# MaurizioFD/RecSys2019_DeepLearning_Evaluation

Hardware: NVIDIA H100
Metric: ItemKNN cosine top-K rows/sec (higher is better)
Workload: dtype i32 counts + f32

## Files before the change

recsys2019_deeplearning_evaluation_b200/csrc/sim_k1d.cuh:

```cuda

constexpr int D_THREADS = 512;
constexpr int D_WARPS = D_THREADS / 32;
constexpr int D_ROWS = 4;
constexpr int D_TILE_LOG2 = 10;

constexpr int K1D_GAPS = 6;
__device__ __forceinline__ int k1d_gap(const int4& c, int e) {
  const int w = e < 2 ? c.y : (e < 4 ? c.z : c.w);
  return (e & 1) ? (int)((unsigned)w >> 16) : (w & 0xffff);
}

struct K1DShared {
  int item, nbuf, cnt, nibsum, tstop, chunk_end, chunk_cnt;
  int ncand, expect;
  CtaSelectSmem<256> sel;
};

__device__ __forceinline__ unsigned nib_ge3(unsigned w) { return (((w | (w >> 1)) >> 2) | (w & (w >> 1))) & 0x11111111u; }
__device__ __forceinline__ unsigned nib_eq2(unsigned w) { return (w >> 1) & ~w & ~(w >> 2) & ~(w >> 3) & 0x11111111u; }
__device__ __forceinline__ unsigned nib_eq1(unsigned w) { return w & ~(w >> 1) & ~(w >> 2) & ~(w >> 3) & 0x11111111u; }
__device__ __forceinline__ unsigned nib_level(unsigned w, int level) {
  return level >= 3 ? nib_ge3(w) : (level == 2 ? nib_eq2(w) : nib_eq1(w));
}
__device__ __forceinline__ int nib_sum(unsigned w) {
// ... 149 lines not shown

    u64 thr = 0ull;
    int n_have = 0;
    const int n3 = ds.ncand;
    const bool collected = n3 <= p.cap_d;
    if (collected) {
      const unsigned* cand = reinterpret_cast<const unsigned*>(buf);
      u64 keys[4];
#pragma unroll
      for (int q = 0; q < 4; ++q) {
        const int t = q * D_THREADS + tid;
        keys[q] = 0ull;
        if (t < n3) {
          const unsigned cd = cand[t];
          const int2 bn = __ldg(p.BN + (cd >> 4));
          const float sv = sim_value<F>(p, (float)(cd & 15u), Ai, __int_as_float(bn.x));
          if (sv > 0.f) keys[q] = (((u64)__float_as_uint(sv)) << 32) | (u64)(0xFFFFFFFFu - (unsigned)bn.y);
        }
      }
      __syncthreads();
#pragma unroll
      for (int q = 0; q < 4; ++q)
        if (keys[q]) buf[atomicAdd(&ds.nbuf, 1)] = keys[q];
      for (int i = tid; i < ntile; i += D_THREADS) tcnt[i] = 0;
      __syncthreads();
      n_have = ds.nbuf;
      if (n_have >= K) {
        const float fl = sim_value<F>(p, 3.f, Ai, tbs[ntile]) * (1.f - 1e-6f);
        if (fl > 0.f) thr = ((u64)__float_as_uint(fl)) << 32;
      }
      PROF_MARK(3);
    }
#pragma unroll 1
    for (int level = collected ? 2 : 3; level >= 1; --level) {
      int t_end = ntile;
      if (level < 3) {
        if (thr == 0ull) {
          t_end = ntile;
        } else {
          const float tsim = __uint_as_float((unsigned)(thr >> 32));
          if (tid == 0) ds.tstop = ntile;
          __syncthreads();
          for (int t = tid; t < ntile; t += D_THREADS)
            if (!(sim_value<F>(p, (float)level, Ai, tbs[t]) >= tsim)) atomicMin(&ds.tstop, t);
          __syncthreads();
          t_end = ds.tstop;
          __syncthreads();
        }
        if (t_end == 0) continue;
        const int w_end = min(Wr, t_end << (D_TILE_LOG2 - 3));
        for (int i = tid; i < w_end; i += D_THREADS) {
          const unsigned w = acc[i];
          if (!w) continue;
          const int c = __popc(nib_level(w, level));
          if (c) atomicAdd(&tcnt[i >> (D_TILE_LOG2 - 3)], c);
        }
        __syncthreads();
      }
      int t0 = 0;
      while (t0 < t_end) {
        if (tid == 0) {
          int t1 = t0, c = 0;
          while (t1 < t_end && n_have + c + tcnt[t1] <= p.cap_d) { c += tcnt[t1]; ++t1; }
          ds.chunk_end = t1;
          ds.chunk_cnt = c;
        }
        __syncthreads();
        const int t1 = ds.chunk_end;
        if (t1 == t0) {
          int kept;
          const u64 t2 = d_select(buf, n_have, K, &ds, &kept);
          thr = max(thr, t2);
          if (tid == 0) ds.nbuf = kept;
          n_have = kept;
          __syncthreads();
          continue;
        }
        if (ds.chunk_cnt > 0) {
          const int w_lo = t0 << (D_TILE_LOG2 - 3), w_hi = min(Wr, t1 << (D_TILE_LOG2 - 3));
          for (int i = w_lo + tid; i < w_hi; i += D_THREADS) {
            const unsigned w = acc[i];
            if (!w) continue;
            unsigned m = nib_level(w, level);
            while (m) {
              const int q = (__ffs(m) - 1) >> 2;
              m &= m - 1;
              const int j = i * 8 + q;
              const float d = (float)((w >> (q << 2)) & 15u);
              const int2 bn = __ldg(p.BN + j);
              const float sv = sim_value<F>(p, d, Ai, __int_as_float(bn.x));
              const u64 key = (((u64)__float_as_uint(sv)) << 32) | (u64)(0xFFFFFFFFu - (unsigned)bn.y);
              if (sv > 0.f && key >= thr) buf[atomicAdd(&ds.nbuf, 1)] = key;
            }
          }
        }
        __syncthreads();
        n_have = ds.nbuf;
        t0 = t1;
      }
      for (int i = tid; i < ntile; i += D_THREADS) tcnt[i] = 0;
      __syncthreads();
      if (n_have >= K) {
        if (level == 3 && thr == 0ull) {
          const float fl = sim_value<F>(p, 3.f, Ai, tbs[ntile]) * (1.f - 1e-6f);
          if (fl > 0.f) thr = ((u64)__float_as_uint(fl)) << 32;
        } else if (level == 2 && n_have > K) {
          int kept;
          const u64 t2 = d_select(buf, n_have, K, &ds, &kept);
          thr = max(thr, t2);
          if (tid == 0) ds.nbuf = kept;
          n_have = kept;
          __syncthreads();
        }
      }
      if (level == 3) PROF_MARK(3); else if (level == 2) PROF_MARK(4); else PROF_MARK(5);
    }

    {
      int kept;
      d_select(buf, n_have, K, &ds, &kept);
      n_have = kept;
    }
    for (int t = tid; t < n_have; t += D_THREADS) {
      const u64 k64 = buf[t];
      emit_entry(p, out_base + t, (int)(0xFFFFFFFFu - (unsigned)k64), __uint_as_float((unsigned)(k64 >> 32)));
    }
    for (int t = n_have + tid; t < K; t += D_THREADS) {
      emit_entry(p, out_base + t, -1, 0.f);
    }
    if (tid == 0) emit_count(p, lc, n_have);
    for (int i = tid; i < (W >> 2); i += D_THREADS) reinterpret_cast<int4*>(acc)[i] = make_int4(0, 0, 0, 0);
    PROF_MARK(6);
  }
}


#ifndef B200_U_THREADS
#define B200_U_THREADS 256
#endif
#ifndef B200_U_CTAS
#define B200_U_CTAS 4
#endif
#ifndef B200_U_STEPS
#define B200_U_STEPS 3
#endif
#ifndef B200_U_STAGE
#define B200_U_STAGE 1024
#endif
constexpr int U_THREADS = B200_U_THREADS;
constexpr int U_WARPS = U_THREADS / 32;
constexpr int U_CTAS = B200_U_CTAS;
constexpr int U_STEPS = B200_U_STEPS;
constexpr int U_STAGE = B200_U_STAGE;

__host__ __device__ __forceinline__ int k1d_window_size(int n, int c) { return ((n - 1) >> 1) + ((n & 1) == 0 && c < (n >> 1) ? 1 : 0); }
__host__ __device__ __forceinline__ int k1d_upper_words(int n) { return (((n >> 1) + 7) / 8 + 3) / 4 * 4; }
constexpr int OWN_SPILLED = (int)0x80000000u;

struct K1DUpShared {
  int item, nibsum, ncand, nst;
  int4 wi;
  unsigned long long base;
};

static_assert(U_STAGE >= 32, "an entry that does not count adds 0 to shared word `lane`");
__device__ __forceinline__ void k1d_up_count(unsigned acc_s, int lane, unsigned t, bool ok) {
  const unsigned word = ok ? t >> 3 : (unsigned)lane, inc = ok ? __funnelshift_l(0u, 1u, t << 2) : 0u;
  asm volatile("red.shared.add.u32 [%0], %1;" :: "r"(acc_s + (word << 2)), "r"(inc) : "memory");
}

__global__ void __launch_bounds__(U_THREADS, U_CTAS) sim_k1d_upper_kernel(const KParams p) {
  extern __shared__ __align__(16) unsigned char smem_raw[];
  __shared__ K1DUpShared us;
  const int tid = threadIdx.x, lane = tid & 31, warp = tid >> 5;
  const int n = p.n_cols;
  const int W = k1d_upper_words(n);
  unsigned* acc = reinterpret_cast<unsigned*>(smem_raw);
  unsigned* stage = acc + W;
  const unsigned acc_s = (unsigned)__cvta_generic_to_shared(acc);
  for (int i = tid; i < W; i += U_THREADS) acc[i] = 0u;
  if (blockIdx.x == 0 && tid == 0 && p.fail_every > 0) atomicExch(p.pair_fail, 1);
  long long prof_t = p.prof ? clock64() : 0;
  if (tid == 0) {
    const int it = atomicAdd(p.counter, 1);
    us.item = *(volatile int*)p.pair_fail ? p.n_range : it;
    if (us.item < p.n_range) us.wi = __ldg(p.worklist_up + us.item);
    us.nibsum = 0; us.ncand = 0; us.nst = 0;
  }
  __syncthreads();

  for (;;) {
    const int item = us.item;
    if (item >= p.n_range) break;
    const int4 wi = us.wi;
    const int col = wi.x, adds = wi.y, cs = wi.z, ce = wi.w;
    const int size_c = k1d_window_size(n, col);
    int it_next = 0, failed = 0;
    if (tid == 0) {
      it_next = atomicAdd(p.counter, 1);
      failed = *(volatile int*)p.pair_fail;
    }

    {
      const unsigned sz = (unsigned)size_c;
      int k0 = cs + warp * 32;
      const auto desc = [&](int k) {
        int2 s = make_int2(0, 0);
        if (k + lane < ce) s = __ldg(p.csc_win + k + lane);
        return s;
      };
      int rstart = 0, beg = 0, end = 0, nr = 0, total = 0, b0 = 0;
      const auto open = [&](int2 seg) {
        const unsigned nz = __ballot_sync(0xffffffffu, seg.y > 0);
        nr = __popc(nz);
        const int src = lane < nr ? (int)__fns(nz, 0, lane + 1) : 0;
        rstart = __shfl_sync(0xffffffffu, seg.x, src);
        const int sy = __shfl_sync(0xffffffffu, seg.y, src);
        const int rn = lane < nr ? sy : 0;
        end = rn;
#pragma unroll
        for (int off = 1; off < 32; off <<= 1) {
          const int t = __shfl_up_sync(0xffffffffu, end, off);
          if (lane >= off) end += t;
        }
        beg = end - rn;
        total = __shfl_sync(0xffffffffu, end, 31);
        b0 = 0;
      };
      bool live = k0 < ce;
      int2 seg_next = make_int2(0, 0);
      if (live) {
        const int2 seg = desc(k0);
        seg_next = desc(k0 + U_WARPS * 32);
        open(seg);
      }
      const auto issue = [&](int4 (&v)[U_STEPS]) {
#pragma unroll
        for (int q = 0; q < U_STEPS; ++q) {
          const int base = b0 + 32 * q, f = base + lane;
          const unsigned before = __ballot_sync(0xffffffffu, lane < nr && end <= base);
          const unsigned ends = __reduce_or_sync(0xffffffffu, (lane < nr && end > base && end - base < 32) ? (1u << (end - base)) : 0u);
          const int row = (__popc(before) + __popc(ends & ((2u << lane) - 1u))) & 31;
          const int rb = __shfl_sync(0xffffffffu, beg, row), rs = __shfl_sync(0xffffffffu, rstart, row);
          v[q] = f < total ? __ldg(p.csr_idx1 + (size_t)rs + (f - rb)) : make_int4(col, 0, 0, 0);
        }
        b0 += 32 * U_STEPS;
        if (b0 >= total) {
          k0 += U_WARPS * 32;
          live = k0 < ce;
          if (live) {
            const int2 seg = seg_next;
            seg_next = desc(k0 + U_WARPS * 32);
            open(seg);
          }
        }
      };
      const auto count = [&](const int4 (&v)[U_STEPS]) {
#pragma unroll
        for (int q = 0; q < U_STEPS; ++q) {
          unsigned t = (unsigned)(v[q].x - col - 1);
          k1d_up_count(acc_s, lane, t, t < sz);
#pragma unroll
          for (int e = 0; e < K1D_GAPS; ++e) {
            const unsigned g = (unsigned)k1d_gap(v[q], e);
            t += g;
            k1d_up_count(acc_s, lane, t, g != 0u && t < sz);
          }
        }
      };
      int4 va[U_STEPS], vb[U_STEPS];
      bool have_a = live;
      if (live) issue(va);
      while (have_a) {
        const bool have_b = live;
        if (live) issue(vb);
        count(va);
        if (!have_b) break;
        have_a = live;
        if (live) issue(va);
        count(vb);
      }
    }
    int4 wi_next = make_int4(0, 0, 0, 0);
    if (tid == 0) {
      it_next = failed ? p.n_range : it_next;
      if (it_next < p.n_range) wi_next = __ldg(p.worklist_up + it_next);
    }
    __syncthreads();
    PROF_MARK(8);

    {
      int ns = 0;
      uint4* acc4 = reinterpret_cast<uint4*>(acc);
      for (int i4 = tid; i4 < ((((size_c + 7) >> 3) + 3) >> 2); i4 += U_THREADS) {
        const uint4 w4 = acc4[i4];
        if (!(w4.x | w4.y | w4.z | w4.w)) continue;
        acc4[i4] = make_uint4(0u, 0u, 0u, 0u);
        const unsigned ww[4] = {w4.x, w4.y, w4.z, w4.w};
        unsigned bytes = 0u, any = 0u, m[4];
#pragma unroll
        for (int e = 0; e < 4; ++e) {
          bytes += (ww[e] & 0x0F0F0F0Fu) + ((ww[e] >> 4) & 0x0F0F0F0Fu);
          m[e] = nib_ge3(ww[e]);
          any |= m[e];
        }
        ns += (int)__dp4a(bytes, 0x01010101u, 0u);
        if (any) {
          const int c3 = __popc(m[0]) + __popc(m[1]) + __popc(m[2]) + __popc(m[3]);
          int pos = atomicAdd(&us.ncand, c3);
          const bool staged = pos + c3 <= U_STAGE;
          unsigned long long g = 0ull;
          if (staged) atomicAdd(&us.nst, c3);
          else g = atomicAdd(p.n_loose, (unsigned long long)c3);
#pragma unroll
          for (int e = 0; e < 4; ++e) {
            unsigned mm = m[e];
            while (mm) {
              const int q = (__ffs(mm) - 1) >> 2;
              mm &= mm - 1;
              int j = col + 1 + (i4 * 4 + e) * 8 + q;
              if (j >= n) j -= n;
              const unsigned cd = ((unsigned)j << 4) | ((ww[e] >> (q << 2)) & 15u);
              if (staged) {
                stage[pos++] = cd;
              } else {
                atomicAdd(p.deg + j, 1);
                if (g < (unsigned long long)p.loose_cap) p.loose[g] = ((u64)col << 32) | cd;
                else atomicExch(p.pair_fail, 1);
                ++g;
              }
            }
          }
        }
      }
      ns = __reduce_add_sync(0xffffffffu, ns);
      if (lane == 0 && ns) atomicAdd(&us.nibsum, ns);
    }
    if (tid == 0) { us.item = it_next; us.wi = wi_next; }
    __syncthreads();
    const int nst = us.nst;
    if (tid == 0) {
      if (us.nibsum != adds) atomicExch(p.pair_fail, 1);
      us.base = nst ? atomicAdd(p.n_own, (unsigned long long)nst) : 0ull;
      if (us.base + nst > (unsigned long long)p.pair_cap) atomicExch(p.pair_fail, 1);
      p.own_off[col] = (int)us.base;
      p.own_n[col] = nst | (us.ncand > nst ? OWN_SPILLED : 0);
    }
    __syncthreads();
    const unsigned long long base = us.base;
    if (base + nst <= (unsigned long long)p.pair_cap)
      for (int t = tid; t < nst; t += U_THREADS) {
        const unsigned cd = stage[t];
        p.own[base + t] = cd;
        atomicAdd(p.deg + (cd >> 4), 1);
      }
    if (tid == 0) { us.nibsum = 0; us.ncand = 0; us.nst = 0; }
    PROF_MARK(9);
  }
}

__global__ void k1d_pair_scatter_kernel(const KParams p) {
  const long long t0 = blockIdx.x * (long long)blockDim.x + threadIdx.x, nt = (long long)gridDim.x * blockDim.x;
  if (*p.pair_fail) {
    for (long long q = t0; q <= p.n_cols; q += nt) p.deg[q] = 0;
    return;
  }
  const int i = (int)(t0 >> 5), lane = threadIdx.x & 31;
  if (i < p.n_cols) {
    const int s = p.own_off[i], n = p.own_n[i] & ~OWN_SPILLED;
    for (int t = lane; t < n; t += 32) {
      const unsigned cd = p.own[s + t], j = cd >> 4;
      p.mir[p.mir_off[j] + atomicSub(p.deg + j, 1) - 1] = ((unsigned)i << 4) | (cd & 15u);
    }
  }
  const long long nl = (long long)min(*p.n_loose, (u64)p.loose_cap);
  for (long long q = t0; q < nl; q += nt) {
    const u64 e = p.loose[q];
    const unsigned cd = (unsigned)e, j = cd >> 4;
    p.mir[p.mir_off[j] + atomicSub(p.deg + j, 1) - 1] = ((unsigned)(e >> 32) << 4) | (cd & 15u);
  }
}

constexpr int S_WARPS = 4;
constexpr int S_CTAS = 6;
constexpr int S_CAP = 4 * D_THREADS;
constexpr int S_ILP = 12;
__host__ __device__ __forceinline__ int k1d_select_warp_bytes(int sel_cap) { return 256 * 4 + (sel_cap * 8 + 15) / 16 * 16; }

template <int F>
__global__ void __launch_bounds__(32 * S_WARPS, S_CTAS) sim_k1d_select_kernel(const KParams p) {
  extern __shared__ __align__(16) unsigned char smem_raw[];
  unsigned char* mine = smem_raw + (size_t)(threadIdx.x >> 5) * k1d_select_warp_bytes(p.sel_cap);
  int* hist = reinterpret_cast<int*>(mine);
  u64* keys = reinterpret_cast<u64*>(mine + 256 * 4);
  const int lane = threadIdx.x & 31;
  const int item = blockIdx.x * S_WARPS + (threadIdx.x >> 5);
  if (item >= p.n_range) return;
  const int4 wi = __ldg(p.worklist + item);
  if (*(volatile int*)p.pair_fail) {
    if (lane == 0) { p.wl_redo[item] = wi; atomicAdd(p.n_redo, 1); }
    return;
  }
  long long prof_t = p.prof ? clock64() : 0;
  const int col = wi.x, lc = wi.y, K = p.K;
  const int so = p.own_off[col], no = p.own_n[col];
  const int sm = p.mir_off[col], n = no + (p.mir_off[col + 1] - sm);
  bool ok = no >= 0 && n <= p.sel_cap;
  int n_have = 0;
  if (ok) {
    const float Ai = p.A[col];
    const unsigned* own = p.own + so;
    const unsigned* mir = p.mir + sm - no;
    for (int t0 = 0; t0 < n; t0 += 32 * S_ILP) {
      unsigned cd[S_ILP];
      int2 bn[S_ILP];
#pragma unroll
      for (int q = 0; q < S_ILP; ++q) {
        const int t = t0 + 32 * q + lane;
        cd[q] = t < n ? (t < no ? own : mir)[t] : 0u;
      }
#pragma unroll
      for (int q = 0; q < S_ILP; ++q)
        if (t0 + 32 * q + lane < n) bn[q] = __ldg(p.BN + (cd[q] >> 4));
#pragma unroll
      for (int q = 0; q < S_ILP; ++q) {
        u64 key = 0ull;
        if (t0 + 32 * q + lane < n) {
          const float sv = sim_value<F>(p, (float)(cd[q] & 15u), Ai, __int_as_float(bn[q].x));
          if (sv > 0.f) key = (((u64)__float_as_uint(sv)) << 32) | (u64)(0xFFFFFFFFu - (unsigned)bn[q].y);
        }
        const unsigned b = __ballot_sync(0xffffffffu, key != 0ull);
        if (key) keys[n_have + __popc(b & ((1u << lane) - 1u))] = key;
        n_have += __popc(b);
      }
    }
    ok = false;
    if (n_have >= K) {
      const float fl = sim_value<F>(p, 3.f, Ai, p.tbnd[p.ntile]) * (1.f - 1e-6f);
      if (fl > 0.f) ok = !(sim_value<F>(p, 2.f, Ai, p.lvl_b2) >= fl) && !(sim_value<F>(p, 1.f, Ai, p.lvl_b1) >= fl);
    }
  }
  PROF_MARK_WARP(10);
  if (!ok) {
    if (lane == 0) p.wl_redo[atomicAdd(p.n_redo, 1)] = wi;
    return;
  }
  __syncwarp();
  const auto sel_key = [&](int q, u64& key) {
    key = keys[q];
    return true;
  };
  const u64 thr = n_have > K ? radix_select<u64, 8, true>(WarpSelect{hist}, n_have, K, sel_key).thr : 0ull;
  const size_t out_base = (size_t)lc * K;
  int kept = 0;
  for (int t0 = 0; t0 < n_have; t0 += 32) {
    const int t = t0 + lane;
    const u64 k64 = t < n_have ? keys[t] : 0ull;
    const bool keep = t < n_have && k64 >= thr;
    const unsigned b = __ballot_sync(0xffffffffu, keep);
    if (keep)
      emit_entry(p, out_base + kept + __popc(b & ((1u << lane) - 1u)), (int)(0xFFFFFFFFu - (unsigned)k64),
                 __uint_as_float((unsigned)(k64 >> 32)));
    kept += __popc(b);
  }
  for (int t = kept + lane; t < K; t += 32) emit_entry(p, out_base + t, -1, 0.f);
  if (lane == 0) emit_count(p, lc, kept);
  PROF_MARK_WARP(11);
}

__global__ void k1d_tile_bounds_kernel(const int2* __restrict__ BN, int n_cols, int ntile, float* tb) {
  const int t = blockIdx.x * blockDim.x + threadIdx.x;
  if (t > ntile) return;
  tb[t] = __int_as_float(BN[min(t << D_TILE_LOG2, n_cols - 1)].x);
}

__device__ __forceinline__ int k1d_row_entry(const int* __restrict__ row, int len, int n_cols, int m) {
  return m < len ? row[m] : row[m - len] + n_cols;
}

template <class Emit>
__device__ __forceinline__ int k1d_row_chunks(const int* __restrict__ row, int len, int copies, int n_cols, Emit emit) {
  const int total = copies * len;
  int nch = 0;
  for (int m = 0; m < total; ++nch) {
    const int base = k1d_row_entry(row, len, n_cols, m++);
    unsigned long long g14 = 0ull;
    unsigned g56 = 0u;
    for (int e = 0, prev = base; e < K1D_GAPS && m < total; ++e, ++m) {
      const int j = k1d_row_entry(row, len, n_cols, m);
      if (j - prev >= 65536) break;
      if (e < 4) g14 |= (unsigned long long)(j - prev) << (16 * e); else g56 |= (unsigned)(j - prev) << (16 * (e - 4));
      prev = j;
    }
    emit(nch, make_int4(base, (int)(unsigned)g14, (int)(unsigned)(g14 >> 32), (int)g56));
  }
  return nch;
}

__global__ void k1d_row_len_kernel(const int* __restrict__ csr_ptr, const int* __restrict__ csr_idx, int n_rows, int copies, int n_cols,
                                   int* nchunk) {
  const int u = blockIdx.x * blockDim.x + threadIdx.x;
  if (u >= n_rows) return;
  nchunk[u] = k1d_row_chunks(csr_idx + csr_ptr[u], csr_ptr[u + 1] - csr_ptr[u], copies, n_cols, [](int, int4) {});
}

__global__ void k1d_row_fill_kernel(const int* __restrict__ csr_ptr, const int* __restrict__ csr_idx, const int* __restrict__ poff,
                                    int n_rows, int copies, int n_cols, int4* rows) {
  const int u = (int)((blockIdx.x * (long long)blockDim.x + threadIdx.x) >> 3), l = threadIdx.x & 7;
  if (u >= n_rows) return;
// ... 60 lines not shown
```

recsys2019_deeplearning_evaluation_b200/csrc/sim_topk.cu:

```cuda
#include <cub/device/device_radix_sort.cuh>
#include <cub/device/device_scan.cuh>
#include <cub/device/device_segmented_sort.cuh>

#include <stdlib.h>

#include <algorithm>
#include <cfloat>
#include <cmath>
#include <cstring>
#include <vector>

#include "common.cuh"
#include "select.cuh"

namespace b200 {
namespace sim {

typedef unsigned long long u64;

constexpr int THREADS = 1024;
constexpr int NWARPS = THREADS / 32;
constexpr int STAGE_INTS = 3072;
constexpr int SPMAX = 5;
constexpr int HBINS = 4096;
// ... 1284 lines not shown
  auto windows_needed = [&](int cells_per_word, long long* cells_out) {
    int nw = 1;
    long long mc = 0;
    for (;; ++nw) {
      const size_t fixed = (size_t)cap * 8 + staging + (size_t)nw * (MAXTILES + 1) * 4 + sizeof(Shared) + 1024;
      mc = (((long long)max_smem - (long long)fixed) / 4) * cells_per_word;
      mc = std::min<long long>(mc, (long long)MAXTILES * THREADS * 4 * cells_per_word);
      B200_REQUIRE(mc >= 4096, "not enough shared memory (%d bytes) for the similarity kernel", max_smem);
      if ((long long)nw * mc >= n_cols) break;
    }
    *cells_out = mc;
    return nw;
  };
  long long max_cells = 0, max_cells_unpacked = 0;
  const int n_win_unpacked = windows_needed(1, &max_cells_unpacked);
  if (h->pack && windows_needed(2, &max_cells) >= n_win_unpacked) h->pack = false;
  const int cpw = h->pack ? 2 : 1;
  const int cpv = 4 * cpw;
  const int tile = THREADS * cpv;
  int n_win = windows_needed(cpw, &max_cells);
  int win = (n_cols + n_win - 1) / n_win;
  win = (win + cpv - 1) / cpv * cpv;
  if (win < cpv) win = cpv;
  h->n_win = n_win;
  h->win = win;
  h->acc_words = std::max(win / cpw, SBINS) + 4;
  h->smem_bytes = (size_t)h->acc_words * 4 + (size_t)cap * 8 + staging + (size_t)n_win * (MAXTILES + 1) * 4;
  raise_smem_limit(kernel_for(h->formula, h->binary, h->pack), h->smem_bytes);
  h->tileB.alloc((size_t)n_win * (MAXTILES + 1));
  tile_bounds_kernel<<<div_up((long long)n_win * (MAXTILES + 1), 128), 128, 0, st>>>(h->BN.get(), n_cols, n_win, win, tile, h->tileB.get());
  count_launch();
  {
    const double avg_seg = nnz > 0 ? (double)nnz / (double)n_rows / (double)n_win : 1.0;
    const double chunks = avg_seg / (h->binary ? 4.0 : 2.0) + 1.0;
    int l2 = 1;
    while (l2 < 5 && (1 << l2) < chunks) ++l2;
    h->lpu_log2 = l2;
  }
  if (n_win > 1 || h->binary) {
    h->split.alloc((size_t)n_rows * (n_win + 1));
    const long long total = (long long)n_rows * (n_win + 1);
    split_kernel<<<div_up(total, 256), 256, 0, st>>>(h->csr_ptr.get(), h->csr_idx.get(), n_rows, n_win, win, h->split.get()); count_launch();
  }
  DevBuf<unsigned long long> win_work;
  DevBuf<int> win_iota;
  if (h->binary) {
    const long long n_seg = (long long)n_rows * n_win;
    B200_REQUIRE((long long)nnz + 3 * n_seg < (1ll << 31), "matrix too large for 32-bit positions in the padded row layout");
    DevBuf<int> len4((size_t)n_seg + 1), poff((size_t)n_seg + 1);
    B200_CUDA(cudaMemsetAsync(len4.get() + n_seg, 0, sizeof(int), st));
    seg_len_kernel<<<div_up(n_seg, 256), 256, 0, st>>>(h->split.get(), n_seg, n_win, len4.get()); count_launch();
    size_t tb = 0;
    B200_CUDA(cub::DeviceScan::ExclusiveSum(nullptr, tb, len4.get(), poff.get(), (int)(n_seg + 1), st));
    DevBuf<unsigned char> tmp(tb);
    B200_CUDA(cub::DeviceScan::ExclusiveSum(tmp.get(), tb, len4.get(), poff.get(), (int)(n_seg + 1), st)); count_launch();
    int total_pad = 0;
    B200_CUDA(cudaMemcpyAsync(&total_pad, poff.get() + n_seg, sizeof(int), cudaMemcpyDeviceToHost, st));
    B200_CUDA(cudaStreamSynchronize(st));
    DevBuf<int> idx_pad((size_t)total_pad + 8), split_pad((size_t)n_rows * (n_win + 1));
    seg_pad_kernel<<<div_up(n_seg * 8, 256), 256, 0, st>>>(h->split.get(), h->csr_idx.get(), poff.get(), n_seg, n_win, win, total_pad,
                                                          idx_pad.get(), split_pad.get()); count_launch();
    B200_CUDA(cudaStreamSynchronize(st));
    const bool f_ok_c = h->formula == F_PROD || h->formula == F_NONORM || h->formula == F_JACCARD || h->formula == F_DICE ||
                        (h->formula == F_TVERSKY && h->ta >= 0.f && h->tb >= 0.f);
    if (h->want_k1c && f_ok_c && nnz > 0 && n_cols >= h->k1c_min_cols) {
      const int copies = 2 * (long long)nnz + 3ll * n_rows < (1ll << 31) ? 2 : 1;
      DevBuf<int> len1((size_t)n_rows + 1), poff1((size_t)n_rows + 1);
      B200_CUDA(cudaMemsetAsync(len1.get() + n_rows, 0, sizeof(int), st));
      k1d_row_len_kernel<<<div_up(n_rows, 256), 256, 0, st>>>(h->csr_ptr.get(), h->csr_idx.get(), n_rows, copies, n_cols, len1.get());
      count_launch();
      size_t tb1 = 0;
      B200_CUDA(cub::DeviceScan::ExclusiveSum(nullptr, tb1, len1.get(), poff1.get(), n_rows + 1, st));
      DevBuf<unsigned char> tmp1(tb1 + 16);
      B200_CUDA(cub::DeviceScan::ExclusiveSum(tmp1.get(), tb1, len1.get(), poff1.get(), n_rows + 1, st)); count_launch();
      int total1 = 0;
      B200_CUDA(cudaMemcpyAsync(&total1, poff1.get() + n_rows, sizeof(int), cudaMemcpyDeviceToHost, st));
      B200_CUDA(cudaStreamSynchronize(st));
      h->csr_idx1.alloc((size_t)total1 + 2);
      k1d_row_fill_kernel<<<div_up((long long)n_rows * 8, 256), 256, 0, st>>>(h->csr_ptr.get(), h->csr_idx.get(), poff1.get(), n_rows,
                                                                             copies, n_cols, h->csr_idx1.get()); count_launch();
      h->col_adds.alloc((size_t)n_cols);
      h->csc_seg.alloc((size_t)nnz + 2);
      B200_CUDA(cudaMemsetAsync(h->csc_seg.get() + nnz, 0, 2 * sizeof(int2), st));
      if (copies == 2) {
        h->csc_win.alloc((size_t)nnz);
        win_work.alloc((size_t)n_cols);
        win_iota.alloc((size_t)n_cols);
      }
      k1d_csc_rows_kernel<<<div_up((long long)n_cols * 32, 256), 256, 0, st>>>(h->csc_ptr.get(), h->csc_idx.get(), h->csr_ptr.get(),
                                                                               h->csr_idx.get(), csc_pos.get(), poff1.get(),
                                                                               h->csr_idx1.get(), n_cols, h->csc_seg.get(),
                                                                               h->col_adds.get(), h->csc_win.get(), win_work.get(),
                                                                               win_iota.get()); count_launch();
      B200_CUDA(cudaStreamSynchronize(st));
    }
    h->csr_idx = std::move(idx_pad);
    h->split = std::move(split_pad);
  }
  csc_pos.release();
  {
    DevBuf<unsigned long long> work((size_t)n_cols);
    col_work_kernel<<<div_up((long long)n_cols * 32, 256), 256, 0, st>>>(h->csc_ptr.get(), h->binary ? h->csc_idx.get() : nullptr,
                                                                        h->binary ? nullptr : h->csc_ent.get(), h->csr_ptr.get(), n_cols, work.get());
    count_launch();
    std::vector<unsigned long long> w_new((size_t)n_cols);
    std::vector<int> o2n((size_t)n_cols);
    B200_CUDA(cudaMemcpyAsync(w_new.data(), work.get(), sizeof(unsigned long long) * (size_t)n_cols, cudaMemcpyDeviceToHost, st));
    B200_CUDA(cudaMemcpyAsync(o2n.data(), h->old2new.get(), sizeof(int) * (size_t)n_cols, cudaMemcpyDeviceToHost, st));
    B200_CUDA(cudaStreamSynchronize(st));
    h->h_work.resize((size_t)n_cols);
    for (int c = 0; c < n_cols; ++c) h->h_work[(size_t)c] = w_new[(size_t)o2n[(size_t)c]];
  }
  if (!h->binary) h->csr_idx.release();
  h->counter.alloc(1);
  h->order.alloc((size_t)n_cols);
  h->k1c = false;
  if (h->csc_seg.n > 0) {
    const int win1 = ((n_cols + 7) / 8) * 8;
    h->ntile = (n_cols + (1 << D_TILE_LOG2) - 1) >> D_TILE_LOG2;
    h->bm_words = ((win1 / 8 + 1) + 3) / 4 * 4;
    const long long fixed = (long long)h->bm_words * 4 + ((long long)h->ntile + 1) * 4 + (long long)h->ntile * 4 + 32;
    cudaFuncAttributes fa{};
    B200_CUDA(cudaFuncGetAttributes(&fa, k1d_kernel_for(h->formula)));
    int dev = 0, sm_total = 0;
    B200_CUDA(cudaGetDevice(&dev));
    B200_CUDA(cudaDeviceGetAttribute(&sm_total, cudaDevAttrMaxSharedMemoryPerMultiprocessor, dev));
    const long long need_keys = (long long)h->K + (1ll << D_TILE_LOG2) + 128;
    for (int ctas = 2; ctas >= 1 && !h->k1c; --ctas) {
      long long avail = (long long)sm_total / ctas - (long long)fa.sharedSizeBytes - 1024;
      avail = std::min<long long>(avail, (long long)max_smem - (long long)fa.sharedSizeBytes);
      const long long keys = std::min<long long>((avail - fixed) / 8, 4 * D_THREADS);
      if (keys >= need_keys) {
        h->ctas_per_sm = ctas;
        h->cap_d = (int)keys;
        h->smem1_bytes = (size_t)(fixed + keys * 8);
        h->k1c = true;
      }
    }
    if (h->k1c) {
      h->tbnd.alloc((size_t)h->ntile + 1);
      k1d_tile_bounds_kernel<<<div_up(h->ntile + 1, 128), 128, 0, st>>>(h->BN.get(), n_cols, h->ntile, h->tbnd.get()); count_launch();
      h->fail.alloc(1);
      h->worklist.alloc((size_t)n_cols);
      h->h_old2new.resize((size_t)n_cols);
      h->h_csc_ptr.resize((size_t)n_cols + 1);
      B200_CUDA(cudaMemcpyAsync(h->h_old2new.data(), h->old2new.get(), sizeof(int) * (size_t)n_cols, cudaMemcpyDeviceToHost, st));
      B200_CUDA(cudaMemcpyAsync(h->h_csc_ptr.data(), h->csc_ptr.get(), sizeof(int) * ((size_t)n_cols + 1), cudaMemcpyDeviceToHost, st));
      B200_CUDA(cudaStreamSynchronize(st));
      raise_smem_limit(k1d_kernel_for(h->formula), h->smem1_bytes);
      B200_CUDA(cudaFuncSetAttribute(k1d_kernel_for(h->formula), cudaFuncAttributePreferredSharedMemoryCarveout, (int)cudaSharedmemCarveoutMaxShared));

      cudaFuncAttributes fu{};
      B200_CUDA(cudaFuncGetAttributes(&fu, sim_k1d_upper_kernel));
      h->smem_up_bytes = ((size_t)k1d_upper_words(n_cols) + U_STAGE) * 4;
      h->ctas_up = 0;
      for (int ctas = U_CTAS; ctas >= 1 && h->ctas_up == 0 && h->csc_win.n > 0; --ctas)
        if ((long long)h->smem_up_bytes <= std::min<long long>((long long)sm_total / ctas - 1024, (long long)max_smem) - (long long)fu.sharedSizeBytes)
          h->ctas_up = ctas;
      if (h->ctas_up > 0 && !k1d_pair_gate(h, cnt_new.get(), st)) h->ctas_up = 0;
      if (h->ctas_up > 0) {
        raise_smem_limit(sim_k1d_upper_kernel, h->smem_up_bytes);
        B200_CUDA(cudaFuncSetAttribute(sim_k1d_upper_kernel, cudaFuncAttributePreferredSharedMemoryCarveout, (int)cudaSharedmemCarveoutMaxShared));
        h->smem_sel_bytes = (size_t)S_WARPS * k1d_select_warp_bytes(h->sel_cap);
        B200_CUDA(cudaFuncSetAttribute(k1d_select_kernel_for(h->formula), cudaFuncAttributeMaxDynamicSharedMemorySize, S_WARPS * k1d_select_warp_bytes(S_CAP)));
        B200_CUDA(cudaFuncSetAttribute(k1d_select_kernel_for(h->formula), cudaFuncAttributePreferredSharedMemoryCarveout, (int)cudaSharedmemCarveoutMaxShared));
        h->worklist_up.alloc((size_t)n_cols);
        DevBuf<unsigned long long> keys_out((size_t)n_cols);
        DevBuf<int> perm((size_t)n_cols);
        size_t tb = 0;
        B200_CUDA(cub::DeviceRadixSort::SortPairsDescending(nullptr, tb, win_work.get(), keys_out.get(), win_iota.get(), perm.get(), n_cols, 0, 64, st));
        DevBuf<unsigned char> tmp(tb + 16);
        B200_CUDA(cub::DeviceRadixSort::SortPairsDescending(tmp.get(), tb, win_work.get(), keys_out.get(), win_iota.get(), perm.get(), n_cols, 0, 64, st));
        k1d_upper_worklist_kernel<<<div_up(n_cols, 256), 256, 0, st>>>(perm.get(), keys_out.get(), h->csc_ptr.get(), n_cols, h->worklist_up.get());
        count_launch(5);
        B200_CUDA(cudaStreamSynchronize(st));
      }
    }
  }
  if (!h->k1c) { h->csr_idx1.release(); h->csc_seg.release(); h->col_adds.release(); }
  if (h->ctas_up == 0) h->csc_win.release();
}

}

extern "C" {

int b200_sim_create(b200_sim_t* out, int64_t n_rows, int64_t n_cols, int64_t nnz, const int32_t* h_indptr,
                    const int32_t* h_indices, const float* h_data, int kind, int topK, float shrink, int normalize,
                    float asymmetric_alpha, float tversky_alpha, float tversky_beta, const float* h_row_weights,
                    void* stream) {
  if (out) *out = nullptr;
  b200_sim_s* h = nullptr;
  int rc = guarded([&] {
    B200_REQUIRE(out != nullptr, "b200_sim_create: out is NULL");
    B200_REQUIRE(n_rows > 0 && n_cols > 0 && nnz >= 0, "b200_sim_create: bad shape %lld x %lld nnz %lld",
                 (long long)n_rows, (long long)n_cols, (long long)nnz);
    B200_REQUIRE(n_rows < (1ll << 31) - 1 && n_cols < (1ll << 31) - 1 && nnz < (1ll << 31) - 1,
                 "b200_sim_create: int32 index range exceeded");
    B200_REQUIRE(kind >= B200_SIM_COSINE && kind <= B200_SIM_TVERSKY, "b200_sim_create: unknown similarity kind %d", kind);
    B200_REQUIRE(topK >= 1, "b200_sim_create: topK must be >= 1 (dense output goes through b200_sim_compute_dense)");
    B200_REQUIRE(h_indptr && (nnz == 0 || (h_indices && h_data)), "b200_sim_create: NULL input array");
    h = new b200_sim_s();
    h->allow_pack = getenv("B200REC_NO_PACK") == nullptr;
    if (const char* e = getenv("B200REC_K1C")) h->want_k1c = atoi(e) != 0;
    if (const char* e = getenv("B200REC_K1C_LAMBDA")) h->k1c_lambda = atof(e);
    if (const char* e = getenv("B200REC_K1C_MINCOLS")) h->k1c_min_cols = atoi(e);
    h->n_rows = (int)n_rows;
    h->n_cols = (int)n_cols;
    h->nnz = nnz;
    h->kind = kind;
    h->K = (int)std::min<int64_t>(topK, n_cols);
    const bool set_kind = kind == B200_SIM_JACCARD || kind == B200_SIM_DICE || kind == B200_SIM_TVERSKY;
    h->normalize = set_kind ? 0 : (normalize != 0);
    h->shrink = shrink;
    h->asym_alpha = asymmetric_alpha;
    h->ta = tversky_alpha;
    h->tb = tversky_beta;
    build(h, h_indptr, h_indices, h_data, h_row_weights, (cudaStream_t)stream);
    *out = h;
  });
  if (rc != B200_OK && h) delete h;
  return rc;
}

int b200_sim_create_scaled(b200_sim_t* out, int64_t n_rows, int64_t n_cols, int64_t nnz, const int32_t* h_indptr,
                           const int32_t* h_indices, const float* h_data, const float* h_A, const float* h_B, int topK,
                           void* stream) {
  if (out) *out = nullptr;
  b200_sim_s* h = nullptr;
  int rc = guarded([&] {
    B200_REQUIRE(out && h_indptr && h_A && h_B && (nnz == 0 || (h_indices && h_data)), "b200_sim_create_scaled: NULL argument");
    B200_REQUIRE(n_rows > 0 && n_cols > 0 && nnz >= 0 && nnz < (1ll << 31) - 1, "b200_sim_create_scaled: bad shape");
    B200_REQUIRE(topK >= 1, "b200_sim_create_scaled: topK must be >= 1");
    h = new b200_sim_s();
    h->n_rows = (int)n_rows; h->n_cols = (int)n_cols; h->nnz = nnz;
    h->kind = B200_SIM_COSINE;
    h->K = (int)std::min<int64_t>(topK, n_cols);
    h->scaled = true;
    h->h_A = h_A; h->h_B = h_B;
    build(h, h_indptr, h_indices, h_data, nullptr, (cudaStream_t)stream);
    h->h_A = h->h_B = nullptr;
    *out = h;
  });
  if (rc != B200_OK && h) delete h;
  return rc;
}

int b200_sim_create_euclidean(b200_sim_t* out, int64_t n_rows, int64_t n_cols, int64_t nnz, const int32_t* h_indptr,
                              const int32_t* h_indices, const float* h_data, int topK, float shrink, int normalize,
                              int normalize_avg_row, int distance_mode, void* stream) {
  if (out) *out = nullptr;
  b200_sim_s* h = nullptr;
  int rc = guarded([&] {
    B200_REQUIRE(out && h_indptr && (nnz == 0 || (h_indices && h_data)), "b200_sim_create_euclidean: NULL argument");
    B200_REQUIRE(n_rows > 0 && n_cols > 0 && nnz >= 0, "b200_sim_create_euclidean: bad shape %lld x %lld nnz %lld",
                 (long long)n_rows, (long long)n_cols, (long long)nnz);
    B200_REQUIRE(n_rows < (1ll << 31) - 1 && n_cols < (1ll << 31) - 1 && nnz < (1ll << 31) - 1,
                 "b200_sim_create_euclidean: int32 index range exceeded");
    B200_REQUIRE(topK >= 1, "b200_sim_create_euclidean: topK must be >= 1");
    B200_REQUIRE(distance_mode >= B200_EUCLID_EXP && distance_mode <= B200_EUCLID_LOG,
                 "b200_sim_create_euclidean: unknown similarity_from_distance_mode %d", distance_mode);
    h = new b200_sim_s();
    h->allow_pack = getenv("B200REC_NO_PACK") == nullptr;
    h->n_rows = (int)n_rows; h->n_cols = (int)n_cols; h->nnz = nnz;
    h->kind = B200_SIM_EUCLIDEAN;
    h->K = (int)std::min<int64_t>(topK, n_cols);
    h->normalize = 0;
    h->shrink = shrink;
    h->eu_mode = distance_mode; h->eu_norm = normalize != 0; h->eu_avg = normalize_avg_row != 0;
    build(h, h_indptr, h_indices, h_data, nullptr, (cudaStream_t)stream);
    *out = h;
  });
  if (rc != B200_OK && h) delete h;
  return rc;
}

int b200_sim_destroy(b200_sim_t h) {
  if (!h) return B200_OK;
  if (h->ev0) cudaEventDestroy(h->ev0);
  if (h->ev1) cudaEventDestroy(h->ev1);
  delete h;
  return B200_OK;
}

int b200_sim_info(b200_sim_t h, int* K, int* n_windows, int* window_cells, int* binary_path, int* signed_data) {
  return guarded([&] {
    B200_REQUIRE(h != nullptr, "b200_sim_info: NULL handle");
    if (K) *K = h->K;
    if (n_windows) *n_windows = h->n_win;
    if (window_cells) *window_cells = h->win;
    if (binary_path) *binary_path = h->binary ? (h->pack ? 2 : 1) : 0;
    if (signed_data) *signed_data = h->signed_data ? 1 : 0;
  });
}

struct PeerOut { int* idx; float* val; int* cnt; };

static void launch_topk(b200_sim_t h, int start_col, int end_col, int32_t* d_idx, float* d_val, int32_t* d_cnt, float* d_dense,
                        cudaStream_t st, const PeerOut* peers = nullptr, int n_peers = 0) {
  const int n_range = end_col - start_col;
  const bool use_k1c = h->k1c && d_dense == nullptr;
  if (h->order_lo != start_col || h->order_hi != end_col || h->order_k1c != use_k1c) {
    const unsigned long long* w = h->h_work.data() + start_col;
    std::vector<int> sparse;
    h->h_order.clear();
    int n_nonempty_dense = 0;
    for (int i = 0; i < n_range; ++i) {
      const bool sp = use_k1c && w[i] > 0 && (double)w[i] <= h->k1c_lambda * (double)h->n_cols;
      (sp ? sparse : h->h_order).push_back(i);
      if (!sp && w[i] > 0) ++n_nonempty_dense;
    }
    h->pair_path_last = h->ctas_up > 0 && use_k1c && start_col == 0 && end_col == h->n_cols && n_nonempty_dense == 0 && !sparse.empty();
    auto by_work = [w](int a, int b) { return w[a] > w[b]; };
    std::stable_sort(h->h_order.begin(), h->h_order.end(), by_work);
    std::stable_sort(sparse.begin(), sparse.end(), by_work);
    h->n_dense_last = (int)h->h_order.size();
    h->n_sparse_last = (int)sparse.size();
    if (!h->h_order.empty())
      B200_CUDA(cudaMemcpyAsync(h->order.get(), h->h_order.data(), sizeof(int) * h->h_order.size(), cudaMemcpyHostToDevice, st));
    std::vector<int4> wl(sparse.size());
    for (size_t k = 0; k < sparse.size(); ++k) {
      const int cn = h->h_old2new[(size_t)(start_col + sparse[k])];
      wl[k] = make_int4(cn, sparse[k], h->h_csc_ptr[(size_t)cn], h->h_csc_ptr[(size_t)cn + 1]);
    }
    if (!wl.empty()) B200_CUDA(cudaMemcpyAsync(h->worklist.get(), wl.data(), sizeof(int4) * wl.size(), cudaMemcpyHostToDevice, st));
    B200_CUDA(cudaStreamSynchronize(st));
    h->order_lo = start_col;
    h->order_hi = end_col;
    h->order_k1c = use_k1c;
  }
  const bool pair_path = h->pair_path_last && n_peers == 0;
  const int n_sparse = use_k1c ? h->n_sparse_last : 0, n_dense = use_k1c ? h->n_dense_last : n_range;
  B200_CUDA(cudaMemsetAsync(h->counter.get(), 0, sizeof(int), st));
  KParams p;
  p.n_cols = h->n_cols; p.K = h->K; p.n_win = h->n_win; p.win = h->win; p.cap = h->cap; p.cap_alloc = h->cap_alloc;
  p.acc_cells = h->acc_words;
  p.lpu_log2 = h->lpu_log2;
  p.tileB = h->tileB.get();
  set_formula_params(p, h);
  p.csr_ptr = h->csr_ptr.get(); p.csr_ent = h->csr_ent.get(); p.csr_idx = h->csr_idx.get();
  p.split = h->split.get();
  p.csc_ptr = h->csc_ptr.get(); p.csc_ent = h->csc_ent.get(); p.csc_idx = h->csc_idx.get();
  p.A = h->A.get(); p.BN = h->BN.get(); p.old2new = h->old2new.get();
  p.col_begin = start_col; p.n_range = n_dense;
  p.order = h->order.get();
  p.counter = h->counter.get();
  p.n_out = 1 + n_peers;
  p.o_idx[0] = d_idx; p.o_val[0] = d_val; p.o_cnt[0] = d_cnt;
  for (int r = 0; r < n_peers; ++r) { p.o_idx[1 + r] = peers[r].idx; p.o_val[1 + r] = peers[r].val; p.o_cnt[1 + r] = peers[r].cnt; }
  p.signed_data = (h->signed_data && h->formula != F_EUCLID) ? 1 : 0;
  p.eu_mode = h->eu_mode; p.eu_norm = h->eu_norm; p.eu_signed = h->signed_data ? 1 : 0;
  p.eu_div = h->eu_avg ? (float)h->n_rows : 1.f;
  p.eu_shrink = h->shrink;
  p.dense_out = d_dense;
  p.prof = h->prof_on ? h->prof.get() : nullptr;
  p.bm_words = h->bm_words; p.cap_d = h->cap_d; p.fail_every = h->fail_every; p.ntile = h->ntile; p.tbnd = h->tbnd.get();
  p.csr_idx1 = h->csr_idx1.get(); p.csc_seg = h->csc_seg.get(); p.col_adds = h->col_adds.get(); p.worklist = h->worklist.get();
  p.redo = h->order.get(); p.fail = h->fail.get();
  p.n_range_dev = nullptr;
  p.csc_win = h->csc_win.get(); p.worklist_up = h->worklist_up.get();
  if (pair_path && h->own.n == 0) {
    h->pair_cap = std::min<long long>((long long)(2.0 * h->pairs_expected) + (1 << 16), (1ll << 30) - 1);
    h->loose_cap = h->pair_cap / 4 + (1 << 16);
    h->own.alloc((size_t)h->pair_cap);
    h->loose.alloc((size_t)h->loose_cap);
    h->mir.alloc((size_t)(h->pair_cap + h->loose_cap));
    h->own_off.alloc((size_t)h->n_cols);
    h->own_n.alloc((size_t)h->n_cols);
    h->deg.alloc((size_t)h->n_cols + 1);
    h->mir_off.alloc((size_t)h->n_cols + 1);
    h->pair_ctl.alloc(6);
    h->wl_redo.alloc((size_t)h->n_cols);
    B200_CUDA(cudaMemsetAsync(h->deg.get(), 0, sizeof(int) * ((size_t)h->n_cols + 1), st));
    B200_CUDA(cub::DeviceScan::ExclusiveSum(nullptr, h->scan_tmp_bytes, h->deg.get(), h->mir_off.get(), h->n_cols + 1, st));
    h->scan_tmp.alloc(h->scan_tmp_bytes + 16);
  }
  p.own = h->own.get(); p.own_off = h->own_off.get(); p.own_n = h->own_n.get(); p.pair_cap = h->pair_cap;
  p.n_own = reinterpret_cast<u64*>(h->pair_ctl.get());
  p.pair_fail = h->pair_ctl.get() + 2; p.n_redo = h->pair_ctl.get() + 3;
  p.loose = h->loose.get(); p.n_loose = reinterpret_cast<u64*>(h->pair_ctl.get() + 4); p.loose_cap = h->loose_cap;
  p.deg = h->deg.get(); p.mir_off = h->mir_off.get(); p.mir = h->mir.get(); p.wl_redo = h->wl_redo.get();
  p.sel_cap = h->sel_cap;
  p.lvl_b1 = h->lvl_b1; p.lvl_b2 = h->lvl_b2;
  B200_CUDA(cudaEventRecord(h->ev0, st));
  if (pair_path) {
    B200_CUDA(cudaMemcpyAsync(h->fail.get(), &h->n_dense_last, sizeof(int), cudaMemcpyHostToDevice, st));
    B200_CUDA(cudaMemsetAsync(h->pair_ctl.get(), 0, 6 * sizeof(int), st));
    KParams q = p;
    q.n_range = h->n_cols;
    sim_k1d_upper_kernel<<<std::min(h->n_cols, h->n_sm * h->ctas_up), U_THREADS, h->smem_up_bytes, st>>>(q);
    q.n_range = n_sparse;
    B200_CUDA(cudaGetLastError());
    size_t tb = h->scan_tmp_bytes;
    B200_CUDA(cub::DeviceScan::ExclusiveSum(h->scan_tmp.get(), tb, h->deg.get(), h->mir_off.get(), h->n_cols + 1, st));
    k1d_pair_scatter_kernel<<<div_up((long long)h->n_cols * 32, 256), 256, 0, st>>>(q);
    B200_CUDA(cudaGetLastError());
    k1d_select_kernel_for(h->formula)<<<div_up(n_sparse, S_WARPS), 32 * S_WARPS, h->smem_sel_bytes, st>>>(q);
    B200_CUDA(cudaGetLastError());
    B200_CUDA(cudaMemsetAsync(h->counter.get(), 0, sizeof(int), st));
    q.worklist = h->wl_redo.get();
    q.n_range_dev = p.n_redo;
    k1d_kernel_for(h->formula)<<<std::min(n_sparse, h->n_sm * h->ctas_per_sm), D_THREADS, h->smem1_bytes, st>>>(q);
    B200_CUDA(cudaGetLastError());
    count_launch(6);
    B200_CUDA(cudaMemsetAsync(h->counter.get(), 0, sizeof(int), st));
    p.n_range_dev = h->fail.get();
  } else if (n_sparse > 0) {
    B200_CUDA(cudaMemcpyAsync(h->fail.get(), &h->n_dense_last, sizeof(int), cudaMemcpyHostToDevice, st));
    KParams q = p;
    q.n_range = n_sparse;
    k1d_kernel_for(h->formula)<<<std::min(n_sparse, h->n_sm * h->ctas_per_sm), D_THREADS, h->smem1_bytes, st>>>(q);
    B200_CUDA(cudaGetLastError());
    count_launch();
    B200_CUDA(cudaMemsetAsync(h->counter.get(), 0, sizeof(int), st));
    p.n_range_dev = h->fail.get();
  }
  if (n_dense > 0 || n_sparse > 0) {
    const int grid = n_sparse > 0 ? h->n_sm : std::min(n_dense, h->n_sm);
    kernel_for(h->formula, h->binary, h->pack)<<<grid, THREADS, h->smem_bytes, st>>>(p);
    B200_CUDA(cudaGetLastError());
    count_launch();
  }
  B200_CUDA(cudaEventRecord(h->ev1, st));
  h->timed = true;
}

int b200_sim_compute_device(b200_sim_t h, int start_col, int end_col, int32_t* d_idx, float* d_val, int32_t* d_cnt,
                            void* stream) {
  return guarded([&] {
    B200_REQUIRE(h != nullptr, "b200_sim_compute: NULL handle");
    B200_REQUIRE(0 <= start_col && start_col <= end_col && end_col <= h->n_cols, "b200_sim_compute: bad column range [%d,%d)",
                 start_col, end_col);
    if (end_col == start_col) return;
    B200_REQUIRE(d_idx && d_val && d_cnt, "b200_sim_compute: NULL output");
    launch_topk(h, start_col, end_col, d_idx, d_val, d_cnt, nullptr, (cudaStream_t)stream);
  });
}

int b200_sim_compute_peers_device(b200_sim_t h, int start_col, int end_col, int n_tables, void* const* d_tables, int64_t idx_offset,
                                  int64_t val_offset, int64_t cnt_offset, void* stream) {
  return guarded([&] {
    B200_REQUIRE(h != nullptr, "b200_sim_compute_peers: NULL handle");
    B200_REQUIRE(0 <= start_col && start_col <= end_col && end_col <= h->n_cols, "b200_sim_compute_peers: bad column range [%d,%d)",
                 start_col, end_col);
    B200_REQUIRE(n_tables >= 1 && n_tables <= B200_MAX_PEERS && d_tables != nullptr, "b200_sim_compute_peers: 1..%d tables", B200_MAX_PEERS);
    if (end_col == start_col) return;
    PeerOut out[B200_MAX_PEERS];
    for (int r = 0; r < n_tables; ++r) {
      B200_REQUIRE(d_tables[r] != nullptr, "b200_sim_compute_peers: NULL table");
      int32_t* base = reinterpret_cast<int32_t*>(d_tables[r]);
      out[r].idx = base + idx_offset + (int64_t)start_col * h->K;
      out[r].val = reinterpret_cast<float*>(base + val_offset) + (int64_t)start_col * h->K;
      out[r].cnt = base + cnt_offset + start_col;
    }
    launch_topk(h, start_col, end_col, out[0].idx, out[0].val, out[0].cnt, nullptr, (cudaStream_t)stream, out + 1, n_tables - 1);
  });
}

int b200_sim_compute_dense_device(b200_sim_t h, int start_col, int end_col, float* d_out, void* stream) {
  return guarded([&] {
    B200_REQUIRE(h != nullptr, "b200_sim_compute_dense: NULL handle");
    B200_REQUIRE(h->formula != F_EUCLID, "b200_sim_compute_dense: the euclidean similarity has no dense output mode");
    B200_REQUIRE(0 <= start_col && start_col <= end_col && end_col <= h->n_cols, "b200_sim_compute_dense: bad column range [%d,%d)",
                 start_col, end_col);
    if (end_col == start_col) return;
    B200_REQUIRE(d_out != nullptr, "b200_sim_compute_dense: NULL output");
    cudaStream_t st = (cudaStream_t)stream;
    B200_CUDA(cudaMemsetAsync(d_out, 0, sizeof(float) * (size_t)(end_col - start_col) * (size_t)h->n_cols, st));
    launch_topk(h, start_col, end_col, nullptr, nullptr, nullptr, d_out, st);
  });
}

int b200_sim_compute(b200_sim_t h, int start_col, int end_col, int32_t* h_idx, float* h_val, int32_t* h_cnt) {
  return guarded([&] {
    B200_REQUIRE(h != nullptr, "b200_sim_compute: NULL handle");
    B200_REQUIRE(0 <= start_col && start_col <= end_col && end_col <= h->n_cols, "b200_sim_compute: bad column range [%d,%d)",
                 start_col, end_col);
    const size_t n_range = (size_t)(end_col - start_col);
    if (n_range == 0) return;
    DevBuf<int> d_idx(n_range * h->K), d_cnt(n_range);
    DevBuf<float> d_val(n_range * h->K);
    int rc = b200_sim_compute_device(h, start_col, end_col, d_idx.get(), d_val.get(), d_cnt.get(), nullptr);
    if (rc != B200_OK) throw CudaFail{rc};
    B200_CUDA(cudaMemcpy(h_idx, d_idx.get(), sizeof(int) * n_range * h->K, cudaMemcpyDeviceToHost));
    B200_CUDA(cudaMemcpy(h_val, d_val.get(), sizeof(float) * n_range * h->K, cudaMemcpyDeviceToHost));
    B200_CUDA(cudaMemcpy(h_cnt, d_cnt.get(), sizeof(int) * n_range, cudaMemcpyDeviceToHost));
  });
}

int b200_sim_debug_set_cap(b200_sim_t h, int cap) {
  return guarded([&] {
    B200_REQUIRE(h != nullptr, "b200_sim_debug_set_cap: NULL handle");
    B200_REQUIRE(cap > h->K && cap <= h->cap_alloc, "b200_sim_debug_set_cap: cap must be in (K, %d]", h->cap_alloc);
    h->cap = cap;
  });
}

int b200_sim_debug_phase_cycles(b200_sim_t h, int enable, uint64_t* out16) {
  return guarded([&] {
    B200_REQUIRE(h != nullptr, "b200_sim_debug_phase_cycles: NULL handle");
    if (h->prof.n == 0) {
      h->prof.alloc(16);
      B200_CUDA(cudaMemset(h->prof.get(), 0, 16 * sizeof(unsigned long long)));
    }
    if (out16) {
      B200_CUDA(cudaDeviceSynchronize());
      B200_CUDA(cudaMemcpy(out16, h->prof.get(), 16 * sizeof(unsigned long long), cudaMemcpyDeviceToHost));
      B200_CUDA(cudaMemset(h->prof.get(), 0, 16 * sizeof(unsigned long long)));
    }
    h->prof_on = enable != 0;
  });
}

int b200_sim_debug_k1c(b200_sim_t h, int set_fail_every, int* enabled, int* ctas_per_sm, int* n_bitmap_cols, int* n_window_cols) {
  return guarded([&] {
    B200_REQUIRE(h != nullptr, "b200_sim_debug_k1c: NULL handle");
// ... 42 lines not shown
```

Baseline: 16.25 million.

## Write upper-triangle candidates straight to global own buffer via per-CTA chunks

Instead of staging candidate pairs in shared memory and copying them to the global own array after a second barrier, each CTA now reserves a chunk of the global own buffer ahead of time and threads write candidates directly into it. Degree atomics are issued inline during candidate extraction. This removes the shared staging area, which shrinks dynamic shared memory and may allow more CTAs per SM, and it drops one syncthreads and the copy loop per item. In exchange the own buffer becomes fragmented, so pair_cap grows by a per-CTA slack term, and the global writes are now scattered per thread rather than a coalesced copy.

```diff
diff --git a/recsys2019_deeplearning_evaluation_b200/csrc/sim_k1d.cuh b/recsys2019_deeplearning_evaluation_b200/csrc/sim_k1d.cuh
--- a/recsys2019_deeplearning_evaluation_b200/csrc/sim_k1d.cuh
+++ b/recsys2019_deeplearning_evaluation_b200/csrc/sim_k1d.cuh
@@ -325,18 +325,19 @@
 constexpr int U_CTAS = B200_U_CTAS;
 constexpr int U_STEPS = B200_U_STEPS;
 constexpr int U_STAGE = B200_U_STAGE;
+constexpr int U_OWN_CHUNK = 4 * U_STAGE;
 
 __host__ __device__ __forceinline__ int k1d_window_size(int n, int c) { return ((n - 1) >> 1) + ((n & 1) == 0 && c < (n >> 1) ? 1 : 0); }
 __host__ __device__ __forceinline__ int k1d_upper_words(int n) { return (((n >> 1) + 7) / 8 + 3) / 4 * 4; }
+__host__ __device__ __forceinline__ int k1d_upper_smem_words(int n) { return max(k1d_upper_words(n), 32); }
 constexpr int OWN_SPILLED = (int)0x80000000u;
 
 struct K1DUpShared {
-  int item, nibsum, ncand, nst;
+  int item, nibsum, ncand;
+  int cur, cur_end;
   int4 wi;
-  unsigned long long base;
 };
 
-static_assert(U_STAGE >= 32, "an entry that does not count adds 0 to shared word `lane`");
 __device__ __forceinline__ void k1d_up_count(unsigned acc_s, int lane, unsigned t, bool ok) {
   const unsigned word = ok ? t >> 3 : (unsigned)lane, inc = ok ? __funnelshift_l(0u, 1u, t << 2) : 0u;
   asm volatile("red.shared.add.u32 [%0], %1;" :: "r"(acc_s + (word << 2)), "r"(inc) : "memory");
@@ -349,7 +350,6 @@
   const int n = p.n_cols;
   const int W = k1d_upper_words(n);
   unsigned* acc = reinterpret_cast<unsigned*>(smem_raw);
-  unsigned* stage = acc + W;
   const unsigned acc_s = (unsigned)__cvta_generic_to_shared(acc);
   for (int i = tid; i < W; i += U_THREADS) acc[i] = 0u;
   if (blockIdx.x == 0 && tid == 0 && p.fail_every > 0) atomicExch(p.pair_fail, 1);
@@ -358,7 +358,7 @@
     const int it = atomicAdd(p.counter, 1);
     us.item = *(volatile int*)p.pair_fail ? p.n_range : it;
     if (us.item < p.n_range) us.wi = __ldg(p.worklist_up + us.item);
-    us.nibsum = 0; us.ncand = 0; us.nst = 0;
+    us.nibsum = 0; us.ncand = 0; us.cur = 0; us.cur_end = 0;
   }
   __syncthreads();
 
@@ -369,9 +369,11 @@
     const int col = wi.x, adds = wi.y, cs = wi.z, ce = wi.w;
     const int size_c = k1d_window_size(n, col);
     int it_next = 0, failed = 0;
+    long long own_next = -1;
     if (tid == 0) {
       it_next = atomicAdd(p.counter, 1);
       failed = *(volatile int*)p.pair_fail;
+      if (us.cur_end - us.cur < U_STAGE) own_next = (long long)atomicAdd(p.n_own, (unsigned long long)U_OWN_CHUNK);
     }
 
     {
@@ -458,10 +460,15 @@
     if (tid == 0) {
       it_next = failed ? p.n_range : it_next;
       if (it_next < p.n_range) wi_next = __ldg(p.worklist_up + it_next);
+      if (own_next >= 0) {
+        if (own_next + U_OWN_CHUNK <= p.pair_cap) { us.cur = (int)own_next; us.cur_end = (int)own_next + U_OWN_CHUNK; }
+        else atomicExch(p.pair_fail, 1);
+      }
     }
     __syncthreads();
     PROF_MARK(8);
 
+    const int own_lo = us.cur, lim = min(U_STAGE, us.cur_end - own_lo);
     {
       int ns = 0;
       uint4* acc4 = reinterpret_cast<uint4*>(acc);
@@ -478,31 +485,29 @@
           any |= m[e];
         }
         ns += (int)__dp4a(bytes, 0x01010101u, 0u);
-        if (any) {
-          const int c3 = __popc(m[0]) + __popc(m[1]) + __popc(m[2]) + __popc(m[3]);
-          int pos = atomicAdd(&us.ncand, c3);
-          const bool staged = pos + c3 <= U_STAGE;
-          unsigned long long g = 0ull;
-          if (staged) atomicAdd(&us.nst, c3);
-          else g = atomicAdd(p.n_loose, (unsigned long long)c3);
-#pragma unroll
-          for (int e = 0; e < 4; ++e) {
-            unsigned mm = m[e];
-            while (mm) {
-              const int q = (__ffs(mm) - 1) >> 2;
-              mm &= mm - 1;
-              int j = col + 1 + (i4 * 4 + e) * 8 + q;
-              if (j >= n) j -= n;
-              const unsigned cd = ((unsigned)j << 4) | ((ww[e] >> (q << 2)) & 15u);
-              if (staged) {
-                stage[pos++] = cd;
-              } else {
-                atomicAdd(p.deg + j, 1);
-                if (g < (unsigned long long)p.loose_cap) p.loose[g] = ((u64)col << 32) | cd;
-                else atomicExch(p.pair_fail, 1);
-                ++g;
-              }
+        if (!any) continue;
+        const int c3 = __popc(m[0]) + __popc(m[1]) + __popc(m[2]) + __popc(m[3]);
+        int pos = atomicAdd(&us.ncand, c3);
+        unsigned long long g = 0ull;
+        if (pos + c3 > lim) g = atomicAdd(p.n_loose, (unsigned long long)(pos + c3 - max(pos, lim)));
+#pragma unroll
+        for (int e = 0; e < 4; ++e) {
+          unsigned mm = m[e];
+          while (mm) {
+            const int q = (__ffs(mm) - 1) >> 2;
+            mm &= mm - 1;
+            int j = col + 1 + (i4 * 4 + e) * 8 + q;
+            if (j >= n) j -= n;
+            const unsigned cd = ((unsigned)j << 4) | ((ww[e] >> (q << 2)) & 15u);
+            atomicAdd(p.deg + j, 1);
+            if (pos < lim) {
+              p.own[own_lo + pos] = cd;
+            } else {
+              if (g < (unsigned long long)p.loose_cap) p.loose[g] = ((u64)col << 32) | cd;
+              else atomicExch(p.pair_fail, 1);
+              ++g;
             }
+            ++pos;
           }
         }
       }
@@ -511,23 +516,14 @@
     }
     if (tid == 0) { us.item = it_next; us.wi = wi_next; }
     __syncthreads();
-    const int nst = us.nst;
     if (tid == 0) {
       if (us.nibsum != adds) atomicExch(p.pair_fail, 1);
-      us.base = nst ? atomicAdd(p.n_own, (unsigned long long)nst) : 0ull;
-      if (us.base + nst > (unsigned long long)p.pair_cap) atomicExch(p.pair_fail, 1);
-      p.own_off[col] = (int)us.base;
-      p.own_n[col] = nst | (us.ncand > nst ? OWN_SPILLED : 0);
-    }
-    __syncthreads();
-    const unsigned long long base = us.base;
-    if (base + nst <= (unsigned long long)p.pair_cap)
-      for (int t = tid; t < nst; t += U_THREADS) {
-        const unsigned cd = stage[t];
-        p.own[base + t] = cd;
-        atomicAdd(p.deg + (cd >> 4), 1);
-      }
-    if (tid == 0) { us.nibsum = 0; us.ncand = 0; us.nst = 0; }
+      const int nc = us.ncand, no = min(nc, lim);
+      p.own_off[col] = own_lo;
+      p.own_n[col] = no | (nc > no ? OWN_SPILLED : 0);
+      us.cur = own_lo + no;
+      us.nibsum = 0; us.ncand = 0;
+    }
     PROF_MARK(9);
   }
 }
diff --git a/recsys2019_deeplearning_evaluation_b200/csrc/sim_topk.cu b/recsys2019_deeplearning_evaluation_b200/csrc/sim_topk.cu
--- a/recsys2019_deeplearning_evaluation_b200/csrc/sim_topk.cu
+++ b/recsys2019_deeplearning_evaluation_b200/csrc/sim_topk.cu
@@ -1460,7 +1460,7 @@
 
       cudaFuncAttributes fu{};
       B200_CUDA(cudaFuncGetAttributes(&fu, sim_k1d_upper_kernel));
-      h->smem_up_bytes = ((size_t)k1d_upper_words(n_cols) + U_STAGE) * 4;
+      h->smem_up_bytes = (size_t)k1d_upper_smem_words(n_cols) * 4;
       h->ctas_up = 0;
       for (int ctas = U_CTAS; ctas >= 1 && h->ctas_up == 0 && h->csc_win.n > 0; --ctas)
         if ((long long)h->smem_up_bytes <= std::min<long long>((long long)sm_total / ctas - 1024, (long long)max_smem) - (long long)fu.sharedSizeBytes)
@@ -1668,8 +1668,10 @@
   p.n_range_dev = nullptr;
   p.csc_win = h->csc_win.get(); p.worklist_up = h->worklist_up.get();
   if (pair_path && h->own.n == 0) {
-    h->pair_cap = std::min<long long>((long long)(2.0 * h->pairs_expected) + (1 << 16), (1ll << 30) - 1);
-    h->loose_cap = h->pair_cap / 4 + (1 << 16);
+    const long long pairs_cap = (long long)(2.0 * h->pairs_expected) + (1 << 16);
+    const long long grid_up = std::min(h->n_cols, h->n_sm * h->ctas_up);
+    h->pair_cap = std::min<long long>(pairs_cap + 2 * grid_up * U_OWN_CHUNK, (1ll << 30) - 1);
+    h->loose_cap = std::min(pairs_cap, h->pair_cap) / 4 + (1 << 16);
     h->own.alloc((size_t)h->pair_cap);
     h->loose.alloc((size_t)h->loose_cap);
     h->mir.alloc((size_t)(h->pair_cap + h->loose_cap));
```

Measured after the change: 16.34 million, median of 6. Within noise of the previous version (+0.6%).
